# assafmu/wav2letter_pytorch

Hardware: AMD Instinct MI355X
Metric: audio-frames/sec/GPU (fwd+bwd+CTC), Wav2Letter 64-mel x 1000-frame bf16 (higher is better)
Workload: dtype bf16

## Files before the change

include/w2l_hip.h:

```cpp
#ifndef W2L_HIP_H
#define W2L_HIP_H
#include <stdint.h>
#ifdef __cplusplus
extern "C" {
#endif

const char* w2l_last_error(void);
int w2l_abi_version(void);


int w2l_pack_weights(const float* w, int64_t s_co, int64_t s_ci, int64_t s_kw, int Cout, int Cin, int Kw,
                     int CoutP, int CinP, void* w_fwd_hi, void* w_fwd_lo, void* w_dgr_hi, void* w_dgr_lo,
                     void* stream);

int w2l_sgd_pack(float* p, float* g, float* m, int first_step, float lr, float momentum, float weight_decay,
                 int nesterov, int zero_grad, int Cout, int Cin, int Kw, void* w_fwd_hi, void* w_fwd_lo, void* w_dgr_hi,
                 void* w_dgr_lo, void* w_fwd_q, void* w_dgr_q, float q_scale, void* stream);

int w2l_nct_to_ntc(const float* x, int N, int C, int T, int CP, int pad_l, int pad_r, int pad_mode,
                   const int32_t* lens, void* out_hi, void* out_lo, void* stream);

int w2l_pad_cast(const float* g, int N, int T, int C, int CP, int halo, void* out_hi, void* out_lo, float* colsum,
                 void* stream);

// ... 51 lines not shown
typedef struct {
    const void* dy;
    int64_t dy_bstride;
    const void* xp;
    int64_t x_bstride;
    int64_t x_rows_total;
    float* dw;
    int Cin, Cout, Kw, pad_;
} w2l_wgrad_item_t;
#define W2L_WGRAD_GROUP_MAX 8
int w2l_conv1d_wgrad_group(const w2l_wgrad_item_t* items, int nitems, int N, int Tout, int dil, int form, void* stream);
int w2l_wgrad_group_tiles(int Cin, int Cout, int Kw, int form);

void w2l_wgrad_force_plan(int splits, int order);
void w2l_wgrad_deterministic(int on);

int w2l_conv1d_wgrad_tune(const void* dy, int64_t dy_bstride, const void* xp, int64_t x_bstride, int64_t x_rows_total,
                          float* dw_scratch, int N, int Cin, int Cout, int Tout, int Kw, int stride, int dil, int reps,
                          void* stream);

int w2l_wgrad_fp8_needs_zero(int N, int Cin, int Cout, int Tout, int Kw);
int w2l_conv1d_wgrad_fp8(const void* dyq, int64_t dy_bstride, const void* xq, int64_t x_bstride, int64_t x_rows_total,
                         float* dw, int N, int Cin, int Cout, int Tout, int Kw, int dil, float descale,
                         const float* descale_dev, int accumulate, void* stream);
int w2l_conv1d_wgrad_fp8_tune(const void* dyq, int64_t dy_bstride, const void* xq, int64_t x_bstride, int64_t x_rows_total,
                              float* dw_scratch, int N, int Cin, int Cout, int Tout, int Kw, int dil, int reps, void* stream);

int w2l_tune_save(const char* path);
int w2l_tune_load(const char* path);

// ... 157 lines not shown
```

wav2letter_pytorch_amd/_lib.py:

```python
from __future__ import annotations

import ctypes as C
import os

os.environ.setdefault('GPU_MAX_HW_QUEUES', '8')

import torch

_HERE = os.path.dirname(os.path.abspath(__file__))
LIB_PATH = os.environ.get('W2L_LIB') or os.path.join(_HERE, 'libw2l_hip.so')

c_p = C.c_void_p
c_i = C.c_int
c_i64 = C.c_int64
c_u64 = C.c_uint64
c_f = C.c_float


class BnActDesc(C.Structure):
    _fields_ = [
        ('N', C.c_int32), ('T', C.c_int32), ('C', C.c_int32),
        ('y', c_p), ('y_f32', C.c_int32),
        ('scale', c_p), ('shift', c_p), ('mean', c_p), ('invstd', c_p),
        ('y2', c_p), ('scale2', c_p), ('shift2', c_p), ('mean2', c_p), ('invstd2', c_p),
# ... 30 lines not shown
    'w2l_nct_to_ntc': (c_i, [c_p, c_i, c_i, c_i, c_i, c_i, c_i, c_i, c_p, c_p, c_p, c_p]),
    'w2l_pad_cast': (c_i, [c_p, c_i, c_i, c_i, c_i, c_i, c_p, c_p, c_p, c_p]),
    'w2l_conv_stat_tiles': (c_i, [c_i, c_i]),
    'w2l_conv1d_igemm': (c_i, [c_p, c_i64, c_i64, c_p, c_p, c_i, c_i, c_p, c_p, c_i, c_i, c_i, c_i, c_i, c_i, c_i, c_p]),
    'w2l_conv1d_igemm_tune': (c_i, [c_p, c_i64, c_i64, c_p, c_p, c_i, c_p, c_p, c_i, c_i, c_i, c_i, c_i, c_i, c_i, c_i, c_p]),
    'w2l_conv1d_igemm_ws': (c_i, [c_p, c_i64, c_i64, c_p, c_p, c_i, c_i, c_p, c_p, c_i, c_i, c_i, c_i, c_i, c_i, c_i, c_p, c_i64, c_p]),
    'w2l_conv1d_igemm_tune_ws': (c_i, [c_p, c_i64, c_i64, c_p, c_p, c_i, c_p, c_p, c_i, c_i, c_i, c_i, c_i, c_i, c_i, c_i, c_p,
                                       c_i64, c_p]),
    'w2l_conv_splitk_workspace_bytes': (c_i64, [c_i, c_i, c_i]),
    'w2l_conv_streamk_ranges': (c_i, [c_i] * 8 + [c_i64]),
    'w2l_conv_streamk_pieces': (c_i, [c_i, c_i, c_i, c_p, c_i]),
    'w2l_conv_force_tile_config': (None, [c_i]),
    'w2l_conv_force_fp8_config': (None, [c_i]),
    'w2l_wgrad_force_plan': (None, [c_i, c_i]),
    'w2l_wgrad_deterministic': (None, [c_i]),
    'w2l_wgrad_needs_zero': (c_i, [c_i, c_i, c_i, c_i, c_i]),
    'w2l_conv1d_wgrad': (c_i, [c_p, c_i64, c_p, c_i64, c_i64, c_p, c_i, c_i, c_i, c_i, c_i, c_i, c_i, c_i, c_p]),
    'w2l_conv1d_wgrad_ws': (c_i, [c_p, c_i64, c_p, c_i64, c_i64, c_p, c_i, c_i, c_i, c_i, c_i, c_i, c_i, c_i, c_p, c_i64, c_p]),
    'w2l_conv1d_wgrad_tune_ws': (c_i, [c_p, c_i64, c_p, c_i64, c_i64, c_p, c_i, c_i, c_i, c_i, c_i, c_i, c_i, c_i, c_p, c_i64, c_p]),
    'w2l_wgrad_needs_zero_ws': (c_i, [c_i, c_i, c_i, c_i, c_i, c_i64]),
    'w2l_wgrad_workspace_bytes': (c_i64, [c_i, c_i, c_i]),
    'w2l_wgrad_dealt_workspace_bytes': (c_i64, [c_i, c_i, c_i]),
    'w2l_conv1d_wgrad_tune_x': (c_i, [c_p, c_i64, c_p, c_i64, c_i64, c_p, c_i, c_i, c_i, c_i, c_i, c_i, c_i, c_i, c_p, c_i64, c_i, c_p]),
    'w2l_wgrad_needs_zero_x': (c_i, [c_i, c_i, c_i, c_i, c_i, c_i, c_i, c_i64]),
    'w2l_wgrad_dealt_segments': (c_i, [c_i, c_i, c_i, c_p, c_i]),
    'w2l_wgrad_plan': (c_i, [c_i, c_i, c_i, c_i, c_i]),
    'w2l_conv1d_wgrad_group': (c_i, [c_p, c_i, c_i, c_i, c_i, c_i, c_p]),
    'w2l_wgrad_group_tiles': (c_i, [c_i, c_i, c_i, c_i]),
    'w2l_conv1d_wgrad_tune': (c_i, [c_p, c_i64, c_p, c_i64, c_i64, c_p, c_i, c_i, c_i, c_i, c_i, c_i, c_i, c_i, c_p]),
    'w2l_dwconv_fwd': (c_i, [c_p, c_p, c_i, c_p, c_p, c_p, c_i, c_i, c_i, c_i, c_i, c_i, c_p, c_p]),
# ... 362 lines not shown
```

wav2letter_pytorch_amd/csrc/conv_wgrad.hip:

```cpp
#include "conv_wgrad_kernel.h"
#include "../../include/w2l_hip.h"
#include <algorithm>
#include <array>
#include <atomic>
#include <map>
#include <mutex>
#include <tuple>
#include <vector>

namespace {
using namespace w2l_wgrad;

template <int KWB, bool S1, bool SK, int TG = 1, bool M32 = false>
__global__ __launch_bounds__(256 * TG, TG == 1 ? 2 : 1) void conv_wgrad_kernel(WgradParams p) {
    extern __shared__ __attribute__((aligned(1024))) char smem[];
    conv_wgrad_body<KWB, S1, SK, TG, M32>(p, smem);
}

}

extern "C" const unsigned char w2l_wgrad3_hsaco[];
extern "C" const unsigned int w2l_wgrad3_hsaco_len;

namespace {

int wgrad3_function(hipFunction_t* fn, int which ) {
    static std::mutex mu;
    static std::map<int, std::array<hipFunction_t, 2>> loaded;
    int dev = 0;
    W2L_CHECK_HIP(hipGetDevice(&dev));
    std::lock_guard<std::mutex> lock(mu);
    auto it = loaded.find(dev);
    if (it == loaded.end()) {
        hipModule_t mod;
        W2L_CHECK_ARG(w2l_wgrad3_hsaco_len > 0, "conv1d_wgrad: the three-tap code object is missing from this build");
        W2L_CHECK_HIP(hipModuleLoadData(&mod, w2l_wgrad3_hsaco));
        std::array<hipFunction_t, 2> f;
        W2L_CHECK_HIP(hipModuleGetFunction(&f[0], mod, "w2l_wgrad3_kernel"));
        W2L_CHECK_HIP(hipModuleGetFunction(&f[1], mod, "w2l_wgrad3x2_kernel"));
        it = loaded.emplace(dev, f).first;
    }
    *fn = it->second[which];
    return 0;
}

typedef std::tuple<int, int, int, int, int> WShapeKey;
std::map<WShapeKey, int> g_wtuned;
std::mutex g_wtuned_mu;
thread_local int g_force_splits = 0;
thread_local int g_force_order = -1;
constexpr int kDefaultOrder = 1;

constexpr int kStreamK = 2;
constexpr int kTapGroups2 = 4;
constexpr int kMfma32 = 8;
constexpr int kTaps3 = 16;
constexpr int kTaps3MaxDil = 4;
constexpr int kDealt = 32;
constexpr int kAtomicSplit = 64;
constexpr int kOrderMask = 127;
constexpr int kDealtFallbackSplits = 2;
constexpr int kResidentBlocks = 512;
thread_local bool g_last_dealt = false;
std::atomic<int> g_deterministic{0};

struct DealtPerm { int nb; std::vector<unsigned short> perm; };
std::map<std::tuple<int, int, int>, DealtPerm> g_dealt_perms;
std::mutex g_dealt_mu;

bool dealt_geometry_ok(int tiles, int S, int G) {
    if (G < 1 || G > W2L_WGRAD_MAX_RANGES || tiles < 1 || tiles > G) return false;
    const int64_t W = (int64_t)tiles * S;
    return W >= G && W * (G + 2) < (1LL << 31);
}

bool dealt_fill(WgradParams& p, int tiles, int S, int G) {
    if (!dealt_geometry_ok(tiles, S, G)) return false;
    std::lock_guard<std::mutex> lock(g_dealt_mu);
    auto key = std::make_tuple(tiles, S, G);
// ... 28 lines not shown
size_t dealt_ws_need(int tiles, int kwblk, int G) {
    return (size_t)64 * 1024 + (size_t)(G + tiles) * kwblk * BM * BNC * sizeof(float);
}

int plan_splits(int N, int Cin, int Cout, int Tout, int Kw, int* tsteps_out, int* order_out = nullptr) {
    const int kwb = Kw > 1 ? KWB_DEFAULT : 1;
    if (order_out) *order_out = g_force_order >= 0 ? g_force_order : kDefaultOrder;
    {
        const int ts = (Tout + BT - 1) / BT;
        if (tsteps_out) *tsteps_out = ts;
        if (g_force_splits > 0)
            return (g_force_order >= 0 && (g_force_order & kDealt)) || g_force_splits <= N * ts ? g_force_splits : N * ts;
        std::lock_guard<std::mutex> lock(g_wtuned_mu);
        auto it = g_wtuned.find(WShapeKey(N, Cin, Cout, Tout, Kw));
        if (it != g_wtuned.end()) {
            if (order_out && g_force_order < 0) *order_out = it->second >> 16;
            return it->second & 0xffff;
        }
    }
    const int tiles = ((Cout + BM - 1) / BM) * ((Cin + BNC - 1) / BNC) * ((Kw + kwb - 1) / kwb);
    const int tsteps = (Tout + BT - 1) / BT;
    const int total = N * tsteps;
    if (tsteps_out) *tsteps_out = tsteps;
    const double t_step_us = 2.7 * kwb / 2.0;
    const double out_us = (double)Cout * Cin * Kw * 4.0 / 1.3e6;
    int best = 1;
    double best_cost = 1e30;
    for (int s = 1; s <= 32 && s <= total; ++s) {
        const int steps = (total + s - 1) / s;
        if (s > 1 && steps < 4) break;
        const long blocks = (long)tiles * s;
        const long rounds = (blocks + 511) / 512;
        double per_step = t_step_us * (blocks <= 256 ? 0.6 : 1.0);
        double cost = rounds * steps * per_step + (s > 1 ? 0.5 * out_us * s : 0.0);
        if (cost < best_cost * 0.97) { best_cost = cost; best = s; }
    }
    return best;
}

}

extern "C" void w2l_wgrad_deterministic(int on) { g_deterministic.store(on ? 1 : 0, std::memory_order_relaxed); }

extern "C" void w2l_wgrad_force_plan(int splits, int order) {
    g_force_splits = splits > 0 ? splits : 0;
    g_force_order = order >= 0 ? (order & kOrderMask) : -1;
}

extern "C" int w2l_wgrad_plan(int N, int Cin, int Cout, int Tout, int Kw) {
    int order = 0;
    const int splits = plan_splits(N, Cin, Cout, Tout, Kw, nullptr, &order);
    return (order & 0xff) | (splits << 8);
}

extern "C" int w2l_wgrad_needs_zero(int N, int Cin, int Cout, int Tout, int Kw) {
    int order = 0;
    const int splits = plan_splits(N, Cin, Cout, Tout, Kw, nullptr, &order);
    if ((order & kDealt) && !(order & kStreamK)) return 1;
// ... 41 lines not shown
        const int t = sg.w / S;
        o[0] = r; o[1] = t; o[2] = sg.w - t * S; o[3] = sg.w_end - t * S; o[4] = sg.split; o[5] = sg.nsplit;
    }
    return nblk;
}

static bool wgrad_ws_ok(int Cin, int Cout, int Kw, int splits, const void* ws, int64_t ws_bytes) {
    if (ws == nullptr) return false;
    const int kwb = Kw > 1 ? KWB_DEFAULT : 1;
    const size_t tiles = (size_t)((Cout + BM - 1) / BM) * ((Cin + BNC - 1) / BNC) * ((Kw + kwb - 1) / kwb);
    return tiles * sizeof(unsigned) <= kWgradTicketBytes && wgrad_ws_need(Cin, Cout, Kw, splits) <= (size_t)ws_bytes;
}

struct WgradResolved {
    int splits, order, tsteps;
    bool streamk, tg2, m32, taps3, slabs, atomic;
    int kwb, kwblk, kgroups, tiles;
    int G;
    bool needs_zero;
};

static WgradResolved wgrad_resolve(int N, int Cin, int Cout, int Tout, int Kw, int stride, int dil, bool have_ws, int64_t ws_bytes) {
    WgradResolved r;
    r.order = 0;
    r.splits = plan_splits(N, Cin, Cout, Tout, Kw, &r.tsteps, &r.order);
    if (g_deterministic.load(std::memory_order_relaxed)) r.order &= ~kAtomicSplit;
    const int order = r.order;
    int G = 0;
    if ((order & kDealt) && !(order & kStreamK)) { G = r.splits; r.splits = kDealtFallbackSplits; }
    const int total_steps = N * r.tsteps;
    if (r.splits > total_steps) r.splits = total_steps;
    if (r.splits > 1) r.splits = (total_steps + (total_steps + r.splits - 1) / r.splits - 1) / ((total_steps + r.splits - 1) / r.splits);
    r.streamk = (order & kStreamK) && (!have_ws || (order & kAtomicSplit));
    if (r.streamk) r.splits = 1;
    r.tg2 = (order & kTapGroups2) && Kw > 2 && !(r.streamk && stride != 1);
    r.m32 = (order & kMfma32) && !r.streamk && !r.tg2 && stride == 1;
    r.taps3 = (order & kTaps3) && !(order & kMfma32) && !r.streamk && stride == 1 && dil <= kTaps3MaxDil && Kw >= 3;
    r.kwb = r.taps3 ? 3 : (Kw > 1 ? KWB_DEFAULT : 1);
    r.kwblk = r.tg2 ? 2 * r.kwb : r.kwb;
    r.kgroups = (Kw + r.kwblk - 1) / r.kwblk;
    r.tiles = ((Cout + BM - 1) / BM) * ((Cin + BNC - 1) / BNC) * r.kgroups;
    r.G = 0;
    if (G > 0 && !r.streamk && have_ws && dealt_geometry_ok(r.tiles, total_steps, G) &&
        dealt_ws_need(r.tiles, r.kwblk, G) <= (size_t)(ws_bytes > 0 ? ws_bytes : 0) && (size_t)r.tiles * sizeof(unsigned) <= 64 * 1024) {
        r.G = G;
        r.splits = 1;
    }
    r.slabs = r.G > 0 || (r.splits > 1 && have_ws && !(order & kAtomicSplit) && (size_t)r.tiles * sizeof(unsigned) <= 64 * 1024 &&
                          wgrad_ws_need(Cin, Cout, Kw, r.splits) <= (size_t)(ws_bytes > 0 ? ws_bytes : 0));
    r.atomic = r.splits > 1 && !r.slabs;
    r.needs_zero = r.atomic || r.streamk;
    return r;
}

extern "C" int w2l_wgrad_needs_zero_x(int N, int Cin, int Cout, int Tout, int Kw, int stride, int dil, int64_t ws_bytes) {
    return wgrad_resolve(N, Cin, Cout, Tout, Kw, stride, dil, ws_bytes > 0, ws_bytes).needs_zero ? 1 : 0;
}

extern "C" int w2l_wgrad_needs_zero_ws(int N, int Cin, int Cout, int Tout, int Kw, int64_t ws_bytes) {
    return w2l_wgrad_needs_zero_x(N, Cin, Cout, Tout, Kw, 1, 1, ws_bytes);
}

extern "C" int64_t w2l_wgrad_workspace_bytes(int Cin, int Cout, int Kw) {
    return (int64_t)wgrad_ws_need(Cin, Cout, Kw, 32);
}

static int wgrad_dispatch(const WgradParams& p, dim3 grid, bool tg2, bool m32, bool taps3, int kwb, int stride, size_t lds, void* stream) {
    dim3 block(tg2 ? 512 : 256);
    static const size_t lds_pad = getenv("W2L_WGRAD_LDS_PAD") ? (size_t)atoll(getenv("W2L_WGRAD_LDS_PAD")) : 0;
    if (!taps3 && lds + lds_pad <= 160 * 1024) lds += lds_pad;
#define W2L_WGRAD_LAUNCH(K, S1_, SK_)                                                                     \
    do {                                                                                                  \
        W2L_CHECK_HIP(w2l_allow_big_lds((const void*)conv_wgrad_kernel<K, S1_, SK_>));                    \
        hipLaunchKernelGGL((conv_wgrad_kernel<K, S1_, SK_>), grid, block, lds, (hipStream_t)stream, p);   \
    } while (0)
    if (taps3) {
        hipFunction_t fn;
        if (int e = wgrad3_function(&fn, tg2 ? 1 : 0)) return e;
        W2L_CHECK_ARG(lds <= 2 * BT * ROWB + 2 * (size_t)(tg2 ? 88 : 72) * ROWB, "conv1d_wgrad: the three-tap kernel's LDS window is too small");
        void* args[] = {const_cast<WgradParams*>(&p)};
        W2L_CHECK_HIP(hipModuleLaunchKernel(fn, grid.x, grid.y, 1, tg2 ? 512 : 256, 1, 1, 0, (hipStream_t)stream, args, nullptr));
    } else if (m32) {
        if (kwb == 2) {
            W2L_CHECK_HIP(w2l_allow_big_lds((const void*)conv_wgrad_kernel<2, true, false, 1, true>));
            hipLaunchKernelGGL((conv_wgrad_kernel<2, true, false, 1, true>), grid, block, lds, (hipStream_t)stream, p);
        } else {
            W2L_CHECK_HIP(w2l_allow_big_lds((const void*)conv_wgrad_kernel<1, true, false, 1, true>));
            hipLaunchKernelGGL((conv_wgrad_kernel<1, true, false, 1, true>), grid, block, lds, (hipStream_t)stream, p);
        }
    } else if (tg2 && p.streamk) {
        W2L_CHECK_HIP(w2l_allow_big_lds((const void*)conv_wgrad_kernel<2, true, true, 2>));
        hipLaunchKernelGGL((conv_wgrad_kernel<2, true, true, 2>), grid, block, lds, (hipStream_t)stream, p);
    } else if (tg2) {
        if (stride == 1) {
// ... 28 lines not shown
    p.nlayers = 1;
    WgradLayer& l0 = p.layers[0];
    l0.dy = (const bf16_raw*)dy;
    l0.x = (const bf16_raw*)xp;
    l0.dw = dw;
    l0.dy_rows_per_utt = dy_bstride / Cout;
    l0.x_rows_per_utt = x_bstride / Cin;
    l0.x_max_row = x_rows_total - 1;
    l0.Cin = Cin; l0.Cout = Cout; l0.Kw = Kw;
    l0.tiles_m = (Cout + BM - 1) / BM;
    l0.tiles_n = (Cin + BNC - 1) / BNC;
    l0.tile0 = 0;
    p.N = N; p.Tout = Tout; p.stride = stride; p.dil = dil;
    const WgradResolved rs = wgrad_resolve(N, Cin, Cout, Tout, Kw, stride, dil, ws != nullptr, ws_bytes);
    const int order = rs.order, splits = rs.splits;
    const bool tg2 = rs.tg2, m32 = rs.m32, taps3 = rs.taps3;
    const int kwb = rs.kwb, kwblk = rs.kwblk;
    p.tsteps = rs.tsteps;
    p.order = order & 1;
    p.streamk = rs.streamk ? 1 : 0;
    p.total_steps = N * p.tsteps;
    p.steps_per_split = (p.total_steps + splits - 1) / splits;
    p.splits = splits;
    p.accumulate = accumulate;
    p.tickets = rs.slabs ? (unsigned*)ws : nullptr;
    p.slabs = rs.slabs ? (float*)((char*)ws + kWgradTicketBytes) : nullptr;
    p.atomic = rs.atomic;
    l0.kgroups = rs.kgroups;
    p.tiles_total = rs.tiles;
    p.dealt = p.dealt_b = 0;
    const int xr = (BT - 1) * stride + (kwblk - 1) * dil + 1;
// ... 5 lines not shown
    if (rs.G > 0) {
        W2L_CHECK_ARG(dealt_fill(p, rs.tiles, p.total_steps, rs.G), "conv1d_wgrad: no dealt form for %d tiles x %d steps on %d ranges",
                      rs.tiles, p.total_steps, rs.G);
        grid = dim3((unsigned)(p.dealt + p.dealt_b), 1);
        g_last_dealt = true;
    }
    if (p.streamk) {
        const int64_t W = (int64_t)grid.x * p.total_steps;
        W2L_CHECK_ARG(W < (1LL << 31), "conv1d_wgrad: (tile, step) space exceeds 32 bits");
        int64_t g = W / 16;
        const int64_t resident = tg2 ? kResidentBlocks / 2 : kResidentBlocks;
        if (g > resident) g = resident;
        if (g < 1) g = 1;
        grid = dim3((unsigned)g, 1);
    }
    return wgrad_dispatch(p, grid, tg2, m32, taps3, kwb, stride, lds, stream);
}

extern "C" int w2l_wgrad_group_tiles(int Cin, int Cout, int Kw, int form) {
    const int kwb = (form & kTaps3) ? 3 : (Kw > 1 ? KWB_DEFAULT : 1);
    const int kwblk = (form & kTapGroups2) ? 2 * kwb : kwb;
    return ((Cout + BM - 1) / BM) * ((Cin + BNC - 1) / BNC) * ((Kw + kwblk - 1) / kwblk);
}

extern "C" int w2l_conv1d_wgrad_group(const w2l_wgrad_item_t* items, int nitems, int N, int Tout, int dil, int form, void* stream) {
    W2L_CHECK_ARG(items && nitems >= 1 && nitems <= W2L_WGRAD_MAX_LAYERS, "conv1d_wgrad_group: 1..%d layers", W2L_WGRAD_MAX_LAYERS);
    W2L_CHECK_ARG(N > 0 && Tout > 0 && dil > 0, "conv1d_wgrad_group: bad sizes");
    const bool taps3 = (form & kTaps3) != 0, tg2 = (form & kTapGroups2) != 0, m32 = (form & kMfma32) != 0 && !taps3 && !tg2;
    W2L_CHECK_ARG(!(form & (kStreamK | kDealt | kAtomicSplit)), "conv1d_wgrad_group: block forms only (order bits 0, 2, 3, 4)");
    W2L_CHECK_ARG(!taps3 || dil <= kTaps3MaxDil, "conv1d_wgrad_group: the three-tap form takes dilation <= %d", kTaps3MaxDil);
    WgradParams p;
    const int kwb = taps3 ? 3 : KWB_DEFAULT, kwblk = tg2 ? 2 * kwb : kwb;
    int tiles = 0;
    for (int i = 0; i < nitems; ++i) {
        const w2l_wgrad_item_t& it = items[i];
        W2L_CHECK_ARG(it.dy && it.xp && it.dw, "conv1d_wgrad_group: null pointer (layer %d)", i);
        W2L_CHECK_ARG(it.Cin % 64 == 0 && it.Cout % 64 == 0 && it.Cin > 0 && it.Cout > 0 && it.Kw > 0,
                      "conv1d_wgrad_group: channels (%d,%d) must be positive multiples of 64", it.Cin, it.Cout);
        W2L_CHECK_ARG(it.Kw > 1 || kwb == KWB_DEFAULT || taps3, "conv1d_wgrad_group: bad form");
        W2L_CHECK_ARG(it.dy_bstride % it.Cout == 0 && it.x_bstride % it.Cin == 0, "conv1d_wgrad_group: batch strides must be whole rows");
        W2L_CHECK_ARG(it.x_rows_total * (int64_t)it.Cin * 2 < (1LL << 32), "conv1d_wgrad_group: activation buffer exceeds 32-bit byte offsets");
        WgradLayer& l = p.layers[i];
        l.dy = (const bf16_raw*)it.dy;
        l.x = (const bf16_raw*)it.xp;
        l.dw = it.dw;
// ... 15 lines not shown
    W2L_CHECK_ARG((int64_t)tiles * p.total_steps < (1LL << 31), "conv1d_wgrad_group: (tile, step) space exceeds 32 bits");
    p.steps_per_split = p.total_steps;
    p.splits = 1;
    p.accumulate = 0;
    p.atomic = 0;
    p.order = form & 1;
    p.streamk = 0;
    p.slabs = nullptr;
    p.tickets = nullptr;
    p.dealt = p.dealt_b = 0;
    const int xr = (BT - 1) + (kwblk - 1) * dil + 1;
    p.xrows_lds = (xr + 3) & ~3;
    const size_t lds = 2 * BT * ROWB + 2 * (size_t)p.xrows_lds * ROWB;
    W2L_CHECK_ARG(lds <= 160 * 1024, "conv1d_wgrad_group: dilation %d needs %zu bytes of LDS", dil, lds);
    g_last_dealt = false;
    return wgrad_dispatch(p, dim3(tiles, 1), tg2, m32, taps3, kwb, 1, lds, stream);
}

extern "C" int w2l_conv1d_wgrad(const void* dy, int64_t dy_bstride, const void* xp, int64_t x_bstride,
                                int64_t x_rows_total, float* dw, int N, int Cin, int Cout, int Tout, int Kw,
                                int stride, int dil, int accumulate, void* stream) {
    return w2l_conv1d_wgrad_ws(dy, dy_bstride, xp, x_bstride, x_rows_total, dw, N, Cin, Cout, Tout, Kw, stride, dil, accumulate,
                               nullptr, 0, stream);
}

extern "C" int w2l_conv1d_wgrad_tune_x(const void* dy, int64_t dy_bstride, const void* xp, int64_t x_bstride,
                                       int64_t x_rows_total, float* dw_scratch, int N, int Cin, int Cout, int Tout, int Kw,
                                       int stride, int dil, int reps, void* ws, int64_t ws_bytes, int flags, void* stream) {
    const WShapeKey key(N, Cin, Cout, Tout, Kw);
    {
        std::lock_guard<std::mutex> lock(g_wtuned_mu);
// ... 20 lines not shown
        if ((order & kDealt) && !g_last_dealt) return -1.f;
        (void)hipEventRecord(e0, st);
        for (int r = 0; r < n; ++r) {
            if (zero) (void)hipMemsetAsync(dw_scratch, 0, bytes, st);
            w2l_conv1d_wgrad_ws(dy, dy_bstride, xp, x_bstride, x_rows_total, dw_scratch, N, Cin, Cout, Tout, Kw, stride, dil, 0,
                                ws, ws_bytes, stream);
        }
        (void)hipEventRecord(e1, st);
        if (hipEventSynchronize(e1) != hipSuccess) return -1.f;
        float ms = 0.f;
        if (hipEventElapsedTime(&ms, e0, e1) != hipSuccess) return -1.f;
        if (zero) ms = ms * 1.08f + 0.008f * n;
        return ms;
    };
    std::vector<std::pair<float, int>> timed;
    const int variants[] = {0, kTapGroups2, kMfma32, kTaps3, kTaps3 | kTapGroups2};
    static const bool no_taps3 = getenv("W2L_WGRAD_NO_TAPS3") != nullptr;
    for (int vi = 0; vi < 5; ++vi) {
        const int tgbit = variants[vi];
        if ((tgbit == kTapGroups2 && Kw <= 2) || (tgbit == kMfma32 && stride != 1)) continue;
        if ((tgbit & kTaps3) && (no_taps3 || stride != 1 || dil > kTaps3MaxDil || Kw < 3 || ((tgbit & kTapGroups2) && Kw <= 3))) continue;
        const bool has_sk = tgbit == 0 || (tgbit == kTapGroups2 && stride == 1);
        for (int ci = has_sk ? -2 : 0; ci < ncand; ++ci) {
            const bool sk = ci < 0;
            if (sk && ws != nullptr && !(flags & 1)) continue;
            const int s = sk ? 1 : cands[ci >> 1];
            int order = sk ? (kStreamK | (ci & 1) | tgbit) : ((ci & 1) | tgbit);
            if ((sk || s > 1) && ws != nullptr && (flags & 1)) order |= kAtomicSplit;
            if (!sk && (s > total || s > 0xffff || (s > 1 && total / s < 4))) break;
            const float ms = time_plan(s, order, reps);
            if (ms >= 0.f) timed.emplace_back(ms, s | (order << 16));
        }
        if (ws != nullptr) {
            const bool waves8 = (tgbit & kTapGroups2) != 0;
            const int ranges[2] = {waves8 ? kResidentBlocks / 2 : kResidentBlocks, waves8 ? 0 : kResidentBlocks / 2};
// ... 8 lines not shown
    std::sort(timed.begin(), timed.end());
    int best = timed.empty() ? -1 : timed[0].second;
    const int finalists = timed.size() < kFinalists ? (int)timed.size() : kFinalists;
    if (finalists > 1) {
        float total_ms[kFinalists] = {};
        for (int round = 0; round < kFinalRounds; ++round)
            for (int k = 0; k < finalists; ++k) {
                const float ms = time_plan(timed[k].second & 0xffff, timed[k].second >> 16, 4 * reps);
                total_ms[k] += ms >= 0.f ? ms : 1e30f;
            }
        int kb = 0;
        for (int k = 1; k < finalists; ++k)
            if (total_ms[k] < total_ms[kb]) kb = k;
        best = timed[kb].second;
    }
    g_force_splits = 0;
    g_force_order = -1;
    (void)hipEventDestroy(e0);
    (void)hipEventDestroy(e1);
    W2L_CHECK_ARG(best >= 1, "conv1d_wgrad_tune: no candidate ran");
    std::lock_guard<std::mutex> lock(g_wtuned_mu);
    g_wtuned[key] = best;
    return 0;
}

extern "C" int w2l_conv1d_wgrad_tune_ws(const void* dy, int64_t dy_bstride, const void* xp, int64_t x_bstride,
                                        int64_t x_rows_total, float* dw_scratch, int N, int Cin, int Cout, int Tout, int Kw,
                                        int stride, int dil, int reps, void* ws, int64_t ws_bytes, void* stream) {
    return w2l_conv1d_wgrad_tune_x(dy, dy_bstride, xp, x_bstride, x_rows_total, dw_scratch, N, Cin, Cout, Tout, Kw, stride, dil,
                                   reps, ws, ws_bytes, 0, stream);
}

extern "C" int w2l_conv1d_wgrad_tune(const void* dy, int64_t dy_bstride, const void* xp, int64_t x_bstride,
                                     int64_t x_rows_total, float* dw_scratch, int N, int Cin, int Cout, int Tout, int Kw,
                                     int stride, int dil, int reps, void* stream) {
    return w2l_conv1d_wgrad_tune_ws(dy, dy_bstride, xp, x_bstride, x_rows_total, dw_scratch, N, Cin, Cout, Tout, Kw, stride, dil,
                                    reps, nullptr, 0, stream);
}

W2L_DIAG_WGRAD_EXPORTS

void w2l_wgrad_tune_dump(FILE* f) {
    std::lock_guard<std::mutex> lock(g_wtuned_mu);
    for (const auto& kv : g_wtuned) {
        const WShapeKey& k = kv.first;
        fprintf(f, "wgrad %d %d %d %d %d %d %d\n", std::get<0>(k), std::get<1>(k), std::get<2>(k), std::get<3>(k),
                std::get<4>(k), kv.second & 0xffff, kv.second >> 16);
    }
}

bool w2l_wgrad_tune_put(const int* v) {
    if (v[5] < 1 || v[5] > 0xffff || v[0] < 1 || v[3] < 1 || v[6] < 0 || v[6] > kOrderMask || ((v[6] & 8) && (v[6] & 6)) || ((v[6] & 16) && (v[6] & 10)))
        return false;
    const int ts = (v[3] + BT - 1) / BT;
    if (v[6] & kDealt) {
        if ((v[6] & kStreamK) || v[5] > W2L_WGRAD_MAX_RANGES) return false;
    } else if ((int64_t)v[5] > (int64_t)v[0] * ts) return false;
    std::lock_guard<std::mutex> lock(g_wtuned_mu);
    g_wtuned[WShapeKey(v[0], v[1], v[2], v[3], v[4])] = v[5] | (v[6] << 16);
    return true;
}
```

wav2letter_pytorch_amd/csrc/conv_wgrad3_dev.hip:

```cpp
#include "conv_wgrad_kernel.h"

using namespace w2l_wgrad;

#define W2L_WGRAD3_XROWS 72

extern "C" __global__ __launch_bounds__(256, 2) void w2l_wgrad3_kernel(WgradParams p) {
    __shared__ __attribute__((aligned(1024))) char smem[2 * BT * ROWB + 2 * W2L_WGRAD3_XROWS * ROWB];
    conv_wgrad_body<3, true, false, 1, true, true>(p, smem);
}

#define W2L_WGRAD3X2_XROWS 88
extern "C" __global__ __launch_bounds__(512, 2) void w2l_wgrad3x2_kernel(WgradParams p) {
    __shared__ __attribute__((aligned(1024))) char smem[2 * BT * ROWB + 2 * W2L_WGRAD3X2_XROWS * ROWB];
    conv_wgrad_body<3, true, false, 2, true, true>(p, smem);
}
```

wav2letter_pytorch_amd/csrc/replay.hip:

```cpp
#include "common.h"
#include "../../include/w2l_hip.h"
#include <string.h>
#include <mutex>
#include <type_traits>
#include <utility>
#include <vector>

extern "C" int w2l_event_create(void** ev) {
    W2L_CHECK_ARG(ev != nullptr, "event_create: null pointer");
    hipEvent_t e;
    W2L_CHECK_HIP(hipEventCreateWithFlags(&e, hipEventDisableTiming));
    *ev = (void*)e;
    return 0;
}
extern "C" int w2l_event_destroy(void* ev) {
    if (ev != nullptr) W2L_CHECK_HIP(hipEventDestroy((hipEvent_t)ev));
    return 0;
}
extern "C" int w2l_event_record(void* ev, void* stream) {
    W2L_CHECK_ARG(ev != nullptr, "event_record: null event");
    W2L_CHECK_HIP(hipEventRecord((hipEvent_t)ev, (hipStream_t)stream));
    return 0;
}
extern "C" int w2l_stream_wait_event(void* stream, void* ev) {
// ... 124 lines not shown
};
template <auto Fn>
int thunk(const w2l_slot_t* a) {
    using S = Sig<decltype(Fn)>;
    return S::template call<Fn>(a, std::make_index_sequence<(size_t)S::arity>{});
}
struct Entry {
    const char* name;
    int (*fn)(const w2l_slot_t*);
    int arity;
};
#define W2L_E(f) {#f, &thunk<&f>, Sig<decltype(&f)>::arity}
const Entry kEntries[] = {
    W2L_E(w2l_event_record), W2L_E(w2l_stream_wait_event), W2L_E(w2l_stream_wait_stream), W2L_E(w2l_fill_zero),
    W2L_E(w2l_pad_vec_f32), W2L_E(w2l_counter_add), W2L_E(w2l_add_i64_multi), W2L_E(w2l_sgd_small_multi),
    W2L_E(w2l_conv_stats_mode), W2L_E(w2l_wgrad_deterministic),
    W2L_E(w2l_pack_weights), W2L_E(w2l_sgd_pack), W2L_E(w2l_novograd_pack), W2L_E(w2l_nct_to_ntc), W2L_E(w2l_pad_cast),
    W2L_E(w2l_conv1d_igemm), W2L_E(w2l_conv1d_igemm_ws), W2L_E(w2l_conv1d_igemm_fp8), W2L_E(w2l_conv1d_dgrad_bnreduce_ws),
    W2L_E(w2l_conv1d_wgrad), W2L_E(w2l_conv1d_wgrad_ws), W2L_E(w2l_conv1d_wgrad_group), W2L_E(w2l_conv1d_wgrad_fp8),
    W2L_E(w2l_dwconv_fwd), W2L_E(w2l_dwconv_dgrad), W2L_E(w2l_dwconv_wgrad),
    W2L_E(w2l_bn_finalize), W2L_E(w2l_bn_act_fwd), W2L_E(w2l_bn_act_fwd_q), W2L_E(w2l_bn_act_fwd_fin),
    W2L_E(w2l_bn_act_bwd_reduce), W2L_E(w2l_bn_act_bwd_reduce_slots), W2L_E(w2l_bn_bwd_finalize), W2L_E(w2l_bn_act_bwd_apply),
    W2L_E(w2l_bn_act_bwd_apply_amax), W2L_E(w2l_bn_act_bwd_apply_fin), W2L_E(w2l_bn_act_bwd_apply_slots),
    W2L_E(w2l_quantize_e4m3), W2L_E(w2l_quantize_e4m3_dyn),
    W2L_E(w2l_log_softmax_fwd), W2L_E(w2l_log_softmax_bwd), W2L_E(w2l_ctc_loss), W2L_E(w2l_argmax),
    W2L_E(w2l_rccl_all_reduce),
};
constexpr int kNumEntries = (int)(sizeof(kEntries) / sizeof(kEntries[0]));
}

extern "C" int w2l_replay_op(const char* name) {
// ... 25 lines not shown
```

wav2letter_pytorch_amd/engine.py:

```python
from __future__ import annotations

import atexit
import ctypes as C
import math
import os
from dataclasses import dataclass, field
from typing import Callable, List, Optional, Sequence

import torch

from . import _lib
from . import wgrad_groups as WG
from ._lib import BnActDesc, GradSrc, check, lib, ptr, stream_ptr

ACT_NONE, ACT_CLAMP20, ACT_RELU = 0, 1, 2
PAD_ZERO, PAD_REFLECT = 0, 1


def _none():
    return None


class _Volatile(dict):

# ... 328 lines not shown
    st = _side_streams.get(dev.index)
    if st is None:
        from .streams import concurrent_stream
        _lib.poison('side stream created')
        st = concurrent_stream(dev, 'wgrad', main=main)
        _side_streams[dev.index] = st
    return st


WGROUP_MAX = int(os.environ.get('W2L_WGRAD_GROUP_MAX', '3'))
_wgrad_ws = {}
_retired_ws = []
DETERMINISTIC_WGRAD = os.environ.get('W2L_DETERMINISTIC', '0') == '1'
lib.w2l_wgrad_deterministic(int(DETERMINISTIC_WGRAD))
DEALT_WGRAD = os.environ.get('W2L_DEALT_WGRAD', '1') == '1'
DEFER_SPREAD = os.environ.get('W2L_DEFER_SPREAD', 'start')
WGRAD_AFTER_DGRAD = os.environ.get('W2L_WGRAD_AFTER_DGRAD', '0') == '1'
FUSED_BN_REDUCE = os.environ.get('W2L_FUSED_BN_REDUCE', '0')
FUSED_BN_REDUCE_MAX_ROWS = 12288
FOLD_BN_FINALIZE = os.environ.get('W2L_FOLD_BN_FINALIZE', '0') == '1'
FOLD_BN_FWD = os.environ.get('W2L_FOLD_BN_FWD', 'auto')
FOLD_BN_FWD_MAX_ROWS = 12288
FAST_BN_BWD = os.environ.get('W2L_FAST_BN_BWD', '1') == '1'
STAT_SLOTS = int(os.environ.get('W2L_STAT_SLOTS', '8'))


def _wgrad_workspace(dev, cin, cout, kw):
    if DETERMINISTIC_WGRAD:
        need = min(int(lib.w2l_wgrad_workspace_bytes(cin, cout, kw)), SPLITK_WS_CAP)
    else:
# ... 599 lines not shown
        if FAST_BN_BWD and not DETERMINISTIC_WGRAD and batch_stats and not self.precise and dev.type == 'cuda':
            slot_need = sum(STAT_SLOTS * 2 * acts[uc.out_index].CP for uc in ctx['units'] if uc.unit.main.has_bn and uc.unit.res is None)
        bias_need = 0
        if batch_stats:
            for u in self.units:
                for c in (u.main, u.res):
                    if c is not None and c.bias is not None and c.has_bn:
                        bias_need += roundup(c.cout, 64)
        zbuf = zeros(pool_elems + slot_need + bias_need, torch.float32, dev)
        small_pool = zbuf[:pool_elems]
        pool_off = 0
        self._slot_pool = [zbuf[pool_elems: pool_elems + slot_need], 0, {}] if slot_need else None
        self._zero_pool = [zbuf[pool_elems + slot_need:], 0] if bias_need else None
        lib.w2l_conv_stats_mode(STAT_SLOTS if self._slot_pool is not None else 0)
        lib.w2l_wgrad_deterministic(int(DETERMINISTIC_WGRAD))
        act_grads: List[List[tuple]] = [[] for _ in acts]
        if self.head is None:
            last = acts[-1]
            _lib.poison('open stack')
            gp = torch.zeros(N, last.T, last.CP, dtype=torch.float32, device=dev)
            gp[:, :, :last.C] = g_out.float().transpose(1, 2)
            act_grads[len(acts) - 1].append((gp, 0, 0, PAD_ZERO, last.T))
        else:
            self._plan_wgrad_groups(ctx)
            pool_off = self._head_backward(ctx, g_out, small_pool, grads, act_grads)
        self._units_backward(ctx, act_grads, small_pool, pool_off, grads, batch_stats)
        for recs in list(self._wg_pending.values()):
            for r in recs:
                self._wgrad_single(r, grads)
        self._wg_pending.clear()
# ... 744 lines not shown
```

wav2letter_pytorch_amd/replay.py:

```python
from __future__ import annotations

import os
import weakref
from typing import Optional

import numpy as np
import torch

from . import _lib
from ._lib import check, lib, ptr

ENABLED = os.environ.get('W2L_REPLAY', '1') != '0'
WARM_STEPS = int(os.environ.get('W2L_REPLAY_WARM', '2'))
MAX_GROUPS = int(os.environ.get('W2L_REPLAY_MAX_SHAPES', '8'))
MAX_FAILURES = 3
FP8_EAGER_EVERY = 256
FP8_EAGER_STEPS = 10
VERBOSE = os.environ.get('W2L_REPLAY_VERBOSE', '0') == '1'
LENS_RING = 4
TRANSIENT = ('fp8 weight scale', 'kernel plans were measured', 'measuring launches', 'workspace grown', 'created', 'table built',
             'momentum buffer')

_last_backward = [None]
STATS = {'recorded': 0, 'replayed_F': 0, 'replayed_B': 0, 'replayed_O': 0, 'replayed_X': 0, 'poisoned': []}
# ... 76 lines not shown
class StepReplayer:

    def __init__(self, engine):
        self.engine = weakref.ref(engine)
        self.groups = {}
        self.pending: Optional[RecordSet] = None
        self.counter = None
        self.counter_host = 0
        self.clock = 0
        self.after_replayed_O = False
        self.opt_stream = None
        self.first_seen = {}

    def _mode_flags(self):
        from . import engine as E
        return (E.DETERMINISTIC_WGRAD, E.DEALT_WGRAD, E.DEFER_SPREAD, E.WGRAD_AFTER_DGRAD, E.FUSED_BN_REDUCE, E.FOLD_BN_FINALIZE,
                E.FOLD_BN_FWD, E.FAST_BN_BWD, E.STAT_SLOTS, E.FP8_DGRAD, E.FP8_WGRAD, E.WGROUP_MAX, E.AUTOTUNE,
                os.environ.get('W2L_WGRAD_GROUPS', 'auto'))

    def plan_forward(self, x, lens, training, softmax_mode, keep_ctx):
        from . import engine as E
        eng = self.engine()
        if (not ENABLED or eng is None or not training or keep_ctx or not x.is_cuda or x.requires_grad or not torch.is_grad_enabled()
                or eng.head is None or eng.precise or eng.grad_ready is not None or eng.flat_ready is not None
                or eng.backward_done is not None or eng.grad_reduce_start is not None or eng.dropout_counter is not None
                or E.KERNEL_TIMER is not None or E.JOIN_EVENTS is not None or _lib._trace['saved'] or _lib.recording() is not None
                or x.dtype != torch.float32 or not x.is_contiguous() or (lens is not None and lens.is_cuda)
                or E.DEFER_SPREAD != 'start' or torch.cuda.is_current_stream_capturing()):
            return None
        purge_pools()
        defer = eng.defer_wgrad if eng.deferred is not None else 0
# ... 410 lines not shown
```

wav2letter_pytorch_amd/wgrad_groups.py:

```python
from __future__ import annotations

import os
from typing import List, Optional, Sequence, Tuple

FORMS = {
    17: (3, 512, 0.95),
    21: (6, 256, 1.00),
    5: (4, 256, 0.97),
    1: (2, 512, 0.90),
}
MAX_GROUP = 8
THREE_TAP_MAX_DIL = 4


def tiles(cin: int, cout: int, kw: int, form: int) -> int:
    kwblk = FORMS[form][0] if (kw > 1 or form & 16) else 1
    return -(-cout // 128) * -(-cin // 128) * -(-kw // kwblk)


def forms_for(dil: int) -> List[int]:
    return [f for f in FORMS if not (f & 16 and dil > THREE_TAP_MAX_DIL)]


LAUNCH_UNITS = 31.0
FILL_UNITS = 26.0
SPLIT_PENALTY = 1.15


def launch_cost(layers: Sequence[Tuple[int, int, int]], form: int, splits: int = 1) -> float:
    kwblk, slots, speed = FORMS[form]
    n = sum(tiles(ci, co, kw, form) for ci, co, kw in layers) * splits
    rounds = -(-n // slots)
    work = rounds * slots * kwblk / splits / speed
    return work * (SPLIT_PENALTY if splits > 1 else 1.0) + LAUNCH_UNITS + (FILL_UNITS if splits > 1 else 0.0)


# ... 57 lines not shown
```

Baseline: 2.533 million.

## Add two-tap paired wgrad kernel with explicit AGPR allocation as tunable variant

Adds a new precompiled two-tap, tap-group-pair wgrad kernel (w2l_wgrad2x2_kernel) built with an explicit amdgpu-agpr-alloc attribute via an IR-patching script. It becomes a new autotune candidate and group form (order bits 4|8). The goal is better register split between VGPRs and AGPRs for the MFMA accumulators, raising occupancy or cutting spills in weight-gradient convolutions. A fallback non-AGPR tuned plan is recorded so the feature can be switched off by environment variable. This costs extra build complexity and more tuning candidates.

```diff
diff --git a/include/w2l_hip.h b/include/w2l_hip.h
--- a/include/w2l_hip.h
+++ b/include/w2l_hip.h
@@ -89,6 +89,7 @@
 
 void w2l_wgrad_force_plan(int splits, int order);
 void w2l_wgrad_deterministic(int on);
+void w2l_wgrad_agpr2(int on);
 
 int w2l_conv1d_wgrad_tune(const void* dy, int64_t dy_bstride, const void* xp, int64_t x_bstride, int64_t x_rows_total,
                           float* dw_scratch, int N, int Cin, int Cout, int Tout, int Kw, int stride, int dil, int reps,
diff --git a/wav2letter_pytorch_amd/_lib.py b/wav2letter_pytorch_amd/_lib.py
--- a/wav2letter_pytorch_amd/_lib.py
+++ b/wav2letter_pytorch_amd/_lib.py
@@ -68,6 +68,7 @@
     'w2l_conv_force_fp8_config': (None, [c_i]),
     'w2l_wgrad_force_plan': (None, [c_i, c_i]),
     'w2l_wgrad_deterministic': (None, [c_i]),
+    'w2l_wgrad_agpr2': (None, [c_i]),
     'w2l_wgrad_needs_zero': (c_i, [c_i, c_i, c_i, c_i, c_i]),
     'w2l_conv1d_wgrad': (c_i, [c_p, c_i64, c_p, c_i64, c_i64, c_p, c_i, c_i, c_i, c_i, c_i, c_i, c_i, c_i, c_p]),
     'w2l_conv1d_wgrad_ws': (c_i, [c_p, c_i64, c_p, c_i64, c_i64, c_p, c_i, c_i, c_i, c_i, c_i, c_i, c_i, c_i, c_p, c_i64, c_p]),
diff --git a/wav2letter_pytorch_amd/csrc/agpr_alloc.py b/wav2letter_pytorch_amd/csrc/agpr_alloc.py
--- /dev/null
+++ b/wav2letter_pytorch_amd/csrc/agpr_alloc.py
@@ -0,0 +1,46 @@
+import re
+import sys
+
+
+def main(path, specs):
+    want = {}
+    for s in specs:
+        name, val = s.split('=')
+        want[name] = int(val)
+    lines = open(path).read().split('\n')
+    groups = {}
+    for i, ln in enumerate(lines):
+        m = re.match(r'attributes #(\d+) = \{ (.*) \}$', ln)
+        if m:
+            groups[int(m.group(1))] = i
+    nxt = max(groups) + 1 if groups else 0
+    done = {}
+    for i, ln in enumerate(lines):
+        m = re.match(r'define .*@(\w+)\(.*\) [^#]*#(\d+) \{$', ln)
+        if not m or m.group(1) not in want:
+            continue
+        name, g = m.group(1), int(m.group(2))
+        body = re.match(r'attributes #\d+ = \{ (.*) \}$', lines[groups[g]]).group(1)
+        if 'amdgpu-agpr-alloc' in body:
+            sys.exit(f'agpr_alloc: {name}: attribute group #{g} already sets amdgpu-agpr-alloc')
+        v = want[name]
+        lines.append(f'attributes #{nxt} = {{ "amdgpu-agpr-alloc"="{v},{v}" {body} }}')
+        lines[i] = ln[:m.start(2) - 1] + f'#{nxt}' + ln[m.end(2):]
+        done[name] = nxt
+        nxt += 1
+    missing = sorted(set(want) - set(done))
+    if missing:
+        sys.exit(f'agpr_alloc: no kernel definition found for {", ".join(missing)}')
+    open(path, 'w').write('\n'.join(lines))
+    text = '\n'.join(lines)
+    for name, g in done.items():
+        if not re.search(rf'^define .*@{name}\(.*#{g} \{{$', text, re.M) or \
+                not re.search(rf'^attributes #{g} = \{{ "amdgpu-agpr-alloc"="{want[name]},{want[name]}" ', text, re.M):
+            sys.exit(f'agpr_alloc: {name}: attribute not in place')
+        print(f'agpr_alloc: {name}: #{g} "amdgpu-agpr-alloc"="{want[name]},{want[name]}"')
+
+
+if __name__ == '__main__':
+    if len(sys.argv) < 3:
+        sys.exit(__doc__)
+    main(sys.argv[1], sys.argv[2:])
diff --git a/wav2letter_pytorch_amd/csrc/conv_wgrad.hip b/wav2letter_pytorch_amd/csrc/conv_wgrad.hip
--- a/wav2letter_pytorch_amd/csrc/conv_wgrad.hip
+++ b/wav2letter_pytorch_amd/csrc/conv_wgrad.hip
@@ -24,9 +24,10 @@
 
 namespace {
 
+enum { kAgThreeTaps = 0, kAgThreeTapsX2 = 1, kAgTwoTapsX2 = 2 };
 int wgrad3_function(hipFunction_t* fn, int which ) {
     static std::mutex mu;
-    static std::map<int, std::array<hipFunction_t, 2>> loaded;
+    static std::map<int, std::array<hipFunction_t, 3>> loaded;
     int dev = 0;
     W2L_CHECK_HIP(hipGetDevice(&dev));
     std::lock_guard<std::mutex> lock(mu);
@@ -35,9 +36,10 @@
         hipModule_t mod;
         W2L_CHECK_ARG(w2l_wgrad3_hsaco_len > 0, "conv1d_wgrad: the three-tap code object is missing from this build");
         W2L_CHECK_HIP(hipModuleLoadData(&mod, w2l_wgrad3_hsaco));
-        std::array<hipFunction_t, 2> f;
-        W2L_CHECK_HIP(hipModuleGetFunction(&f[0], mod, "w2l_wgrad3_kernel"));
-        W2L_CHECK_HIP(hipModuleGetFunction(&f[1], mod, "w2l_wgrad3x2_kernel"));
+        std::array<hipFunction_t, 3> f;
+        W2L_CHECK_HIP(hipModuleGetFunction(&f[kAgThreeTaps], mod, "w2l_wgrad3_kernel"));
+        W2L_CHECK_HIP(hipModuleGetFunction(&f[kAgThreeTapsX2], mod, "w2l_wgrad3x2_kernel"));
+        W2L_CHECK_HIP(hipModuleGetFunction(&f[kAgTwoTapsX2], mod, "w2l_wgrad2x2_kernel"));
         it = loaded.emplace(dev, f).first;
     }
     *fn = it->second[which];
@@ -46,6 +48,7 @@
 
 typedef std::tuple<int, int, int, int, int> WShapeKey;
 std::map<WShapeKey, int> g_wtuned;
+std::map<WShapeKey, int> g_wtuned_noag2;
 std::mutex g_wtuned_mu;
 thread_local int g_force_splits = 0;
 thread_local int g_force_order = -1;
@@ -54,6 +57,8 @@
 constexpr int kStreamK = 2;
 constexpr int kTapGroups2 = 4;
 constexpr int kMfma32 = 8;
+constexpr int kAgpr2 = kTapGroups2 | kMfma32;
+constexpr int kAgpr2MaxDil = 4;
 constexpr int kTaps3 = 16;
 constexpr int kTaps3MaxDil = 4;
 constexpr int kDealt = 32;
@@ -63,6 +68,7 @@
 constexpr int kResidentBlocks = 512;
 thread_local bool g_last_dealt = false;
 std::atomic<int> g_deterministic{0};
+std::atomic<int> g_agpr2{getenv("W2L_WGRAD_NO_AGPR2") && atoi(getenv("W2L_WGRAD_NO_AGPR2")) ? 0 : 1};
 
 struct DealtPerm { int nb; std::vector<unsigned short> perm; };
 std::map<std::tuple<int, int, int>, DealtPerm> g_dealt_perms;
@@ -121,6 +127,10 @@
         std::lock_guard<std::mutex> lock(g_wtuned_mu);
         auto it = g_wtuned.find(WShapeKey(N, Cin, Cout, Tout, Kw));
         if (it != g_wtuned.end()) {
+            if (!g_agpr2.load(std::memory_order_relaxed) && ((it->second >> 16) & kAgpr2) == kAgpr2) {
+                auto alt = g_wtuned_noag2.find(it->first);
+                if (alt != g_wtuned_noag2.end()) it = alt;
+            }
             if (order_out && g_force_order < 0) *order_out = it->second >> 16;
             return it->second & 0xffff;
         }
@@ -149,6 +159,8 @@
 
 extern "C" void w2l_wgrad_deterministic(int on) { g_deterministic.store(on ? 1 : 0, std::memory_order_relaxed); }
 
+extern "C" void w2l_wgrad_agpr2(int on) { g_agpr2.store(on ? 1 : 0, std::memory_order_relaxed); }
+
 extern "C" void w2l_wgrad_force_plan(int splits, int order) {
     g_force_splits = splits > 0 ? splits : 0;
     g_force_order = order >= 0 ? (order & kOrderMask) : -1;
@@ -220,7 +232,7 @@
 
 struct WgradResolved {
     int splits, order, tsteps;
-    bool streamk, tg2, m32, taps3, slabs, atomic;
+    bool streamk, tg2, m32, taps3, agpr2, slabs, atomic;
     int kwb, kwblk, kgroups, tiles;
     int G;
     bool needs_zero;
@@ -241,6 +253,8 @@
     if (r.streamk) r.splits = 1;
     r.tg2 = (order & kTapGroups2) && Kw > 2 && !(r.streamk && stride != 1);
     r.m32 = (order & kMfma32) && !r.streamk && !r.tg2 && stride == 1;
+    r.agpr2 = (order & kAgpr2) == kAgpr2 && r.tg2 && !r.streamk && stride == 1 && dil <= kAgpr2MaxDil &&
+              g_agpr2.load(std::memory_order_relaxed);
     r.taps3 = (order & kTaps3) && !(order & kMfma32) && !r.streamk && stride == 1 && dil <= kTaps3MaxDil && Kw >= 3;
     r.kwb = r.taps3 ? 3 : (Kw > 1 ? KWB_DEFAULT : 1);
     r.kwblk = r.tg2 ? 2 * r.kwb : r.kwb;
@@ -271,19 +285,21 @@
     return (int64_t)wgrad_ws_need(Cin, Cout, Kw, 32);
 }
 
-static int wgrad_dispatch(const WgradParams& p, dim3 grid, bool tg2, bool m32, bool taps3, int kwb, int stride, size_t lds, void* stream) {
+static int wgrad_dispatch(const WgradParams& p, dim3 grid, bool tg2, bool m32, bool taps3, bool agpr2, int kwb, int stride, size_t lds,
+                          void* stream) {
     dim3 block(tg2 ? 512 : 256);
     static const size_t lds_pad = getenv("W2L_WGRAD_LDS_PAD") ? (size_t)atoll(getenv("W2L_WGRAD_LDS_PAD")) : 0;
-    if (!taps3 && lds + lds_pad <= 160 * 1024) lds += lds_pad;
+    if (!taps3 && !agpr2 && lds + lds_pad <= 160 * 1024) lds += lds_pad;
 #define W2L_WGRAD_LAUNCH(K, S1_, SK_)                                                                     \
     do {                                                                                                  \
         W2L_CHECK_HIP(w2l_allow_big_lds((const void*)conv_wgrad_kernel<K, S1_, SK_>));                    \
         hipLaunchKernelGGL((conv_wgrad_kernel<K, S1_, SK_>), grid, block, lds, (hipStream_t)stream, p);   \
     } while (0)
-    if (taps3) {
+    if (taps3 || agpr2) {
         hipFunction_t fn;
-        if (int e = wgrad3_function(&fn, tg2 ? 1 : 0)) return e;
-        W2L_CHECK_ARG(lds <= 2 * BT * ROWB + 2 * (size_t)(tg2 ? 88 : 72) * ROWB, "conv1d_wgrad: the three-tap kernel's LDS window is too small");
+        if (int e = wgrad3_function(&fn, agpr2 ? kAgTwoTapsX2 : tg2 ? kAgThreeTapsX2 : kAgThreeTaps)) return e;
+        const size_t xrows = agpr2 ? 76 : tg2 ? 88 : 72;
+        W2L_CHECK_ARG(lds <= 2 * BT * ROWB + 2 * xrows * ROWB, "conv1d_wgrad: the AGPR kernel's LDS window is too small");
         void* args[] = {const_cast<WgradParams*>(&p)};
         W2L_CHECK_HIP(hipModuleLaunchKernel(fn, grid.x, grid.y, 1, tg2 ? 512 : 256, 1, 1, 0, (hipStream_t)stream, args, nullptr));
     } else if (m32) {
@@ -342,7 +358,7 @@
     p.N = N; p.Tout = Tout; p.stride = stride; p.dil = dil;
     const WgradResolved rs = wgrad_resolve(N, Cin, Cout, Tout, Kw, stride, dil, ws != nullptr, ws_bytes);
     const int order = rs.order, splits = rs.splits;
-    const bool tg2 = rs.tg2, m32 = rs.m32, taps3 = rs.taps3;
+    const bool tg2 = rs.tg2, m32 = rs.m32, taps3 = rs.taps3, agpr2 = rs.agpr2;
     const int kwb = rs.kwb, kwblk = rs.kwblk;
     p.tsteps = rs.tsteps;
     p.order = order & 1;
@@ -378,7 +394,7 @@
         if (g < 1) g = 1;
         grid = dim3((unsigned)g, 1);
     }
-    return wgrad_dispatch(p, grid, tg2, m32, taps3, kwb, stride, lds, stream);
+    return wgrad_dispatch(p, grid, tg2, m32, taps3, agpr2, kwb, stride, lds, stream);
 }
 
 extern "C" int w2l_wgrad_group_tiles(int Cin, int Cout, int Kw, int form) {
@@ -391,8 +407,11 @@
     W2L_CHECK_ARG(items && nitems >= 1 && nitems <= W2L_WGRAD_MAX_LAYERS, "conv1d_wgrad_group: 1..%d layers", W2L_WGRAD_MAX_LAYERS);
     W2L_CHECK_ARG(N > 0 && Tout > 0 && dil > 0, "conv1d_wgrad_group: bad sizes");
     const bool taps3 = (form & kTaps3) != 0, tg2 = (form & kTapGroups2) != 0, m32 = (form & kMfma32) != 0 && !taps3 && !tg2;
+    const bool agpr2 = (form & kAgpr2) == kAgpr2 && !taps3 && g_agpr2.load(std::memory_order_relaxed);
     W2L_CHECK_ARG(!(form & (kStreamK | kDealt | kAtomicSplit)), "conv1d_wgrad_group: block forms only (order bits 0, 2, 3, 4)");
     W2L_CHECK_ARG(!taps3 || dil <= kTaps3MaxDil, "conv1d_wgrad_group: the three-tap form takes dilation <= %d", kTaps3MaxDil);
+    W2L_CHECK_ARG((form & kAgpr2) != kAgpr2 || dil <= kAgpr2MaxDil, "conv1d_wgrad_group: the two-tap AGPR form takes dilation <= %d",
+                  kAgpr2MaxDil);
     WgradParams p;
     const int kwb = taps3 ? 3 : KWB_DEFAULT, kwblk = tg2 ? 2 * kwb : kwb;
     int tiles = 0;
@@ -438,7 +457,7 @@
     const size_t lds = 2 * BT * ROWB + 2 * (size_t)p.xrows_lds * ROWB;
     W2L_CHECK_ARG(lds <= 160 * 1024, "conv1d_wgrad_group: dilation %d needs %zu bytes of LDS", dil, lds);
     g_last_dealt = false;
-    return wgrad_dispatch(p, dim3(tiles, 1), tg2, m32, taps3, kwb, 1, lds, stream);
+    return wgrad_dispatch(p, dim3(tiles, 1), tg2, m32, taps3, agpr2, kwb, 1, lds, stream);
 }
 
 extern "C" int w2l_conv1d_wgrad(const void* dy, int64_t dy_bstride, const void* xp, int64_t x_bstride,
@@ -489,11 +508,12 @@
         return ms;
     };
     std::vector<std::pair<float, int>> timed;
-    const int variants[] = {0, kTapGroups2, kMfma32, kTaps3, kTaps3 | kTapGroups2};
+    const int variants[] = {0, kTapGroups2, kMfma32, kTaps3, kTaps3 | kTapGroups2, kAgpr2};
     static const bool no_taps3 = getenv("W2L_WGRAD_NO_TAPS3") != nullptr;
-    for (int vi = 0; vi < 5; ++vi) {
+    for (int vi = 0; vi < 6; ++vi) {
         const int tgbit = variants[vi];
         if ((tgbit == kTapGroups2 && Kw <= 2) || (tgbit == kMfma32 && stride != 1)) continue;
+        if (tgbit == kAgpr2 && (!g_agpr2.load(std::memory_order_relaxed) || stride != 1 || dil > kAgpr2MaxDil || Kw <= 2)) continue;
         if ((tgbit & kTaps3) && (no_taps3 || stride != 1 || dil > kTaps3MaxDil || Kw < 3 || ((tgbit & kTapGroups2) && Kw <= 3))) continue;
         const bool has_sk = tgbit == 0 || (tgbit == kTapGroups2 && stride == 1);
         for (int ci = has_sk ? -2 : 0; ci < ncand; ++ci) {
@@ -532,6 +552,10 @@
             if (total_ms[k] < total_ms[kb]) kb = k;
         best = timed[kb].second;
     }
+    int best_noag2 = -1;
+    if (best >= 1 && ((best >> 16) & kAgpr2) == kAgpr2)
+        for (const auto& t : timed)
+            if (((t.second >> 16) & kAgpr2) != kAgpr2) { best_noag2 = t.second; break; }
     g_force_splits = 0;
     g_force_order = -1;
     (void)hipEventDestroy(e0);
@@ -539,6 +563,8 @@
     W2L_CHECK_ARG(best >= 1, "conv1d_wgrad_tune: no candidate ran");
     std::lock_guard<std::mutex> lock(g_wtuned_mu);
     g_wtuned[key] = best;
+    if (best_noag2 >= 1) g_wtuned_noag2[key] = best_noag2;
+    else g_wtuned_noag2.erase(key);
     return 0;
 }
 
@@ -568,7 +594,7 @@
 }
 
 bool w2l_wgrad_tune_put(const int* v) {
-    if (v[5] < 1 || v[5] > 0xffff || v[0] < 1 || v[3] < 1 || v[6] < 0 || v[6] > kOrderMask || ((v[6] & 8) && (v[6] & 6)) || ((v[6] & 16) && (v[6] & 10)))
+    if (v[5] < 1 || v[5] > 0xffff || v[0] < 1 || v[3] < 1 || v[6] < 0 || v[6] > kOrderMask || ((v[6] & 8) && (v[6] & 2)) || ((v[6] & 16) && (v[6] & 10)))
         return false;
     const int ts = (v[3] + BT - 1) / BT;
     if (v[6] & kDealt) {
@@ -576,5 +602,6 @@
     } else if ((int64_t)v[5] > (int64_t)v[0] * ts) return false;
     std::lock_guard<std::mutex> lock(g_wtuned_mu);
     g_wtuned[WShapeKey(v[0], v[1], v[2], v[3], v[4])] = v[5] | (v[6] << 16);
+    g_wtuned_noag2.erase(WShapeKey(v[0], v[1], v[2], v[3], v[4]));
     return true;
 }
diff --git a/wav2letter_pytorch_amd/csrc/conv_wgrad3_dev.hip b/wav2letter_pytorch_amd/csrc/conv_wgrad3_dev.hip
--- a/wav2letter_pytorch_amd/csrc/conv_wgrad3_dev.hip
+++ b/wav2letter_pytorch_amd/csrc/conv_wgrad3_dev.hip
@@ -14,3 +14,9 @@
     __shared__ __attribute__((aligned(1024))) char smem[2 * BT * ROWB + 2 * W2L_WGRAD3X2_XROWS * ROWB];
     conv_wgrad_body<3, true, false, 2, true, true>(p, smem);
 }
+
+#define W2L_WGRAD2X2_XROWS 76
+extern "C" __global__ __launch_bounds__(512, 2) void w2l_wgrad2x2_kernel(WgradParams p) {
+    __shared__ __attribute__((aligned(1024))) char smem[2 * BT * ROWB + 2 * W2L_WGRAD2X2_XROWS * ROWB];
+    conv_wgrad_body<2, true, false, 2, true, true>(p, smem);
+}
diff --git a/wav2letter_pytorch_amd/csrc/replay.hip b/wav2letter_pytorch_amd/csrc/replay.hip
--- a/wav2letter_pytorch_amd/csrc/replay.hip
+++ b/wav2letter_pytorch_amd/csrc/replay.hip
@@ -162,7 +162,7 @@
 const Entry kEntries[] = {
     W2L_E(w2l_event_record), W2L_E(w2l_stream_wait_event), W2L_E(w2l_stream_wait_stream), W2L_E(w2l_fill_zero),
     W2L_E(w2l_pad_vec_f32), W2L_E(w2l_counter_add), W2L_E(w2l_add_i64_multi), W2L_E(w2l_sgd_small_multi),
-    W2L_E(w2l_conv_stats_mode), W2L_E(w2l_wgrad_deterministic),
+    W2L_E(w2l_conv_stats_mode), W2L_E(w2l_wgrad_deterministic), W2L_E(w2l_wgrad_agpr2),
     W2L_E(w2l_pack_weights), W2L_E(w2l_sgd_pack), W2L_E(w2l_novograd_pack), W2L_E(w2l_nct_to_ntc), W2L_E(w2l_pad_cast),
     W2L_E(w2l_conv1d_igemm), W2L_E(w2l_conv1d_igemm_ws), W2L_E(w2l_conv1d_igemm_fp8), W2L_E(w2l_conv1d_dgrad_bnreduce_ws),
     W2L_E(w2l_conv1d_wgrad), W2L_E(w2l_conv1d_wgrad_ws), W2L_E(w2l_conv1d_wgrad_group), W2L_E(w2l_conv1d_wgrad_fp8),
diff --git a/wav2letter_pytorch_amd/engine.py b/wav2letter_pytorch_amd/engine.py
--- a/wav2letter_pytorch_amd/engine.py
+++ b/wav2letter_pytorch_amd/engine.py
@@ -366,6 +366,7 @@
 DETERMINISTIC_WGRAD = os.environ.get('W2L_DETERMINISTIC', '0') == '1'
 lib.w2l_wgrad_deterministic(int(DETERMINISTIC_WGRAD))
 DEALT_WGRAD = os.environ.get('W2L_DEALT_WGRAD', '1') == '1'
+AGPR2_WGRAD = os.environ.get('W2L_WGRAD_NO_AGPR2', '0') != '1'
 DEFER_SPREAD = os.environ.get('W2L_DEFER_SPREAD', 'start')
 WGRAD_AFTER_DGRAD = os.environ.get('W2L_WGRAD_AFTER_DGRAD', '0') == '1'
 FUSED_BN_REDUCE = os.environ.get('W2L_FUSED_BN_REDUCE', '0')
@@ -995,6 +996,7 @@
         self._zero_pool = [zbuf[pool_elems + slot_need:], 0] if bias_need else None
         lib.w2l_conv_stats_mode(STAT_SLOTS if self._slot_pool is not None else 0)
         lib.w2l_wgrad_deterministic(int(DETERMINISTIC_WGRAD))
+        lib.w2l_wgrad_agpr2(int(AGPR2_WGRAD))
         act_grads: List[List[tuple]] = [[] for _ in acts]
         if self.head is None:
             last = acts[-1]
diff --git a/wav2letter_pytorch_amd/replay.py b/wav2letter_pytorch_amd/replay.py
--- a/wav2letter_pytorch_amd/replay.py
+++ b/wav2letter_pytorch_amd/replay.py
@@ -114,7 +114,7 @@
 
     def _mode_flags(self):
         from . import engine as E
-        return (E.DETERMINISTIC_WGRAD, E.DEALT_WGRAD, E.DEFER_SPREAD, E.WGRAD_AFTER_DGRAD, E.FUSED_BN_REDUCE, E.FOLD_BN_FINALIZE,
+        return (E.DETERMINISTIC_WGRAD, E.DEALT_WGRAD, E.AGPR2_WGRAD, E.DEFER_SPREAD, E.WGRAD_AFTER_DGRAD, E.FUSED_BN_REDUCE, E.FOLD_BN_FINALIZE,
                 E.FOLD_BN_FWD, E.FAST_BN_BWD, E.STAT_SLOTS, E.FP8_DGRAD, E.FP8_WGRAD, E.WGROUP_MAX, E.AUTOTUNE,
                 os.environ.get('W2L_WGRAD_GROUPS', 'auto'))
 
diff --git a/wav2letter_pytorch_amd/wgrad_groups.py b/wav2letter_pytorch_amd/wgrad_groups.py
--- a/wav2letter_pytorch_amd/wgrad_groups.py
+++ b/wav2letter_pytorch_amd/wgrad_groups.py
@@ -7,6 +7,7 @@
     17: (3, 512, 0.95),
     21: (6, 256, 1.00),
     5: (4, 256, 0.97),
+    13: (4, 256, 0.97),
     1: (2, 512, 0.90),
 }
 MAX_GROUP = 8
@@ -19,7 +20,7 @@
 
 
 def forms_for(dil: int) -> List[int]:
-    return [f for f in FORMS if not (f & 16 and dil > THREE_TAP_MAX_DIL)]
+    return [f for f in FORMS if not ((f & 16 or (f & 12) == 12) and dil > THREE_TAP_MAX_DIL)]
 
 
 LAUNCH_UNITS = 31.0
```

Result: no change. 2.535 million (median of 6 runs) (+0.1%).
